# African-Robotics-Unit/AcinoSet

Measured on AMD Instinct MI355X. Metric: FTE frames/sec (residual+Jac+LM step), 6-cam x 20-joint, higher is better.
Workload: dtype f64

## Files before the change

### acinoset_amd/csrc/chunk.hip

```cpp
#include "chunk.hpp"

#include <algorithm>
#include <cstdlib>
#include <type_traits>

#include "bcr_dev.hpp"
#include "trio80.hpp"

namespace acino {

void ChunkPlan::build(int nodes_total, int chunk_nodes, bool pin_l, bool pin_r) {
  n_nodes = nodes_total;
  m = n_chunks = n_sep = 0;
  node0 = pin_l ? 1 : 0;
  pin_right = pin_r ? 1 : 0;
  const int nodes = nodes_total - node0;
  if (chunk_nodes < 0 || nodes < 1) return;
  int mm = chunk_nodes;
  if (mm == 0) {
    mm = (nodes + 255) / 256;
    mm = std::max(4, std::min(mm, 512));
  }
  mm = std::max(2, mm);
  m = mm;
  n_chunks = (nodes + mm - 1) / mm;
  if (pin_r && n_chunks > 1 && nodes - (n_chunks - 1) * mm == 1) --n_chunks;
  n_sep = n_chunks - 1 + node0 + pin_right;
}

__device__ __forceinline__ void tile_store(double* M, int ib, int jb, const d4& a, int li, int lk) {
#pragma unroll
  for (int rr = 0; rr < 4; ++rr) M[(ib * 16 + lk + 4 * rr) * LD + jb * 16 + li] = a[rr];
}

constexpr int SW_VEC = 18 * NP + 2 * BS + 8 + 8 + 3 * NP + 64;
static constexpr size_t kSweepLds = (3 * MAT + SW_VEC) * sizeof(double);

__device__ __forceinline__ int opaque(int x) {
  asm volatile("" : "+v"(x));
  return x;
}

__device__ __forceinline__ unsigned opaque_u(unsigned x) {
  asm volatile("" : "+v"(x));
  return x;
}
struct BuildSlot {
  int pr, pc, base, e;
  bool own, dg;
  static __device__ __forceinline__ BuildSlot unpack(unsigned w) {
    BuildSlot s;
    s.pr = w & 31;
    s.pc = (w >> 5) & 31;
    s.own = (w >> 10) & 1;
    s.dg = (w >> 11) & 1;
    s.base = (w >> 12) & 2047;
    s.e = w >> 23;
    return s;
  }
};
static_assert((NP - 1) * LD + NP - 1 < 2048 && 13 * NP <= 512 && NP <= 32, "BuildSlot's bit fields");

constexpr int SW_T = 512;
template <int NQ>
__device__ __forceinline__ void syrk_mask_n(d4 (&acc)[NQ], bool load) {
#pragma unroll
  for (int q = 0; q < NQ; ++q)
#pragma unroll
    for (int rr = 0; rr < 4; ++rr) acc[q][rr] = load ? acc[q][rr] : 0.0;
}
constexpr int SP_STEPS = 4 * NT - 1;
__device__ __forceinline__ void spike_gf(const double* G, const double (&bF)[NT][4], d4 (&acc)[NT], int li, int lk) {
  double a[3][NT];
  const double* gb = G + lk * LD + li;
  auto fetch = [&](int buf, int step) {
#pragma unroll
    for (int ib = 0; ib < NT; ++ib) a[buf][ib] = gb[(4 * step) * LD + ib * 16];
  };
#pragma unroll
  for (int ib = 0; ib < NT; ++ib) acc[ib] = d4{0, 0, 0, 0};
  fetch(0, 0);
  fetch(1, 1);
#pragma unroll
  for (int step = 0; step < SP_STEPS; ++step) {
    if (step + 2 < SP_STEPS) fetch((step + 2) % 3, step + 2);
    __builtin_amdgcn_sched_barrier(0);
#pragma unroll
    for (int ib = 0; ib < NT; ++ib) acc[ib] = mfma(a[step % 3][ib], bF[step >> 2][step & 3], acc[ib]);
    __builtin_amdgcn_sched_barrier(0);
  }
}
template <int NQ>
__device__ __forceinline__ void spike_ftt(d4 (&acc)[NQ], const double* Yf, const d4 (&T)[NT], const int (&as)[NQ], int li, int lk) {
  constexpr int DEPTH = NQ >= 3 ? 2 : (NQ == 2 ? 3 : 6);
  const double* p = Yf + lk * LD + li;
  double a[DEPTH + 1][NQ];
#pragma unroll
  for (int d = 0; d < DEPTH; ++d)
#pragma unroll
    for (int q = 0; q < NQ; ++q) a[d][q] = p[(4 * d) * LD + as[q] * 16];
#pragma unroll
  for (int st = 0; st < SP_STEPS; ++st) {
    if (st + DEPTH < SP_STEPS) {
#pragma unroll
      for (int q = 0; q < NQ; ++q) a[(st + DEPTH) % (DEPTH + 1)][q] = p[(4 * (st + DEPTH)) * LD + as[q] * 16];
    }
    __builtin_amdgcn_sched_barrier(0);
#pragma unroll
    for (int q = 0; q < NQ; ++q) acc[q] = mfma(-a[st % (DEPTH + 1)][q], T[st >> 2][st & 3], acc[q]);
    __builtin_amdgcn_sched_barrier(0);
  }
}
template <int NQ>
struct AlTiles {
  d4 acc[NQ];
  int as[NQ], j;
  double* Ag;
  __device__ __forceinline__ double* at(int q, int rr, int li, int lk) const {
    return as[q] >= j ? Ag + (size_t)(as[q] * 16 + 4 * rr + lk) * BS + j * 16 + li
                      : Ag + (size_t)(j * 16 + li) * BS + as[q] * 16 + 4 * rr + lk;
  }
  __device__ __forceinline__ void fetch(int li, int lk) {
#pragma unroll
    for (int q = 0; q < NQ; ++q)
#pragma unroll
      for (int rr = 0; rr < 4; ++rr) acc[q][rr] = *at(q, rr, li, lk);
  }
  __device__ __forceinline__ void run(bool load, const double* Yf, const d4 (&T)[NT], int li, int lk) {
    syrk_mask_n<NQ>(acc, load);
    spike_ftt<NQ>(acc, Yf, T, as, li, lk);
#pragma unroll
    for (int q = 0; q < NQ; ++q)
#pragma unroll
      for (int rr = 0; rr < 4; ++rr) *at(q, rr, li, lk) = acc[q][rr];
  }
};
__device__ __forceinline__ int role8(int wave) { return (0x75236410u >> (4 * wave)) & 15; }
constexpr int ctri_i(int t) { return (t >= 1) + (t >= 3) + (t >= 6) + (t >= 10); }
template <int T>
struct GramTile {
  static constexpr int ib = ctri_i(T), jb = T - ib * (ib + 1) / 2, ns = 4 * (NT - ib);
};
template <int T>
__device__ __forceinline__ void gram_fetch(const double* X, int li, int lk, double (&a)[GramTile<T>::ns], double (&b)[GramTile<T>::ns]) {
  const double* pa = X + (GramTile<T>::ib * 16 + li) * LD + GramTile<T>::ib * 16 + lk;
  const double* pb = X + (GramTile<T>::jb * 16 + li) * LD + GramTile<T>::ib * 16 + lk;
#pragma unroll
  for (int s = 0; s < GramTile<T>::ns; ++s) {
    a[s] = pa[4 * s];
    b[s] = pb[4 * s];
  }
}
template <int T>
__device__ __forceinline__ void gram_tile(double* Xg, int li, int lk, const double (&a)[GramTile<T>::ns], const double (&b)[GramTile<T>::ns]) {
  constexpr int ib = GramTile<T>::ib, jb = GramTile<T>::jb;
  d4 g = {0, 0, 0, 0};
#pragma unroll
  for (int s = 0; s < GramTile<T>::ns; ++s) g = mfma(a[s], b[s], g);
#pragma unroll
  for (int rr = 0; rr < 4; ++rr) {
    Xg[(ib * 16 + lk + 4 * rr) * LD + jb * 16 + li] = g[rr];
    if (ib != jb) Xg[(jb * 16 + li) * LD + ib * 16 + lk + 4 * rr] = g[rr];
  }
}
template <int T0, int... REST>
__device__ __forceinline__ void gram_chain(const double* Xf, double* Xg, int li, int lk, const double (&a)[GramTile<T0>::ns],
                                           const double (&b)[GramTile<T0>::ns]) {
  if constexpr (sizeof...(REST) > 0) {
    constexpr int rest[] = {REST...};
    double an[GramTile<rest[0]>::ns], bn[GramTile<rest[0]>::ns];
    gram_fetch<rest[0]>(Xf, li, lk, an, bn);
    __builtin_amdgcn_sched_barrier(0);
    gram_tile<T0>(Xg, li, lk, a, b);
    __builtin_amdgcn_sched_barrier(0);
    gram_chain<REST...>(Xf, Xg, li, lk, an, bn);
  } else {
    gram_tile<T0>(Xg, li, lk, a, b);
  }
}
template <int T0, int... REST>
__device__ __forceinline__ void gram_fixed(const double* Xf, double* Xg, int* done, int li, int lk, int lane) {
  double a[GramTile<T0>::ns], b[GramTile<T0>::ns];
  gram_fetch<T0>(Xf, li, lk, a, b);
  gram_chain<T0, REST...>(Xf, Xg, li, lk, a, b);
  asm volatile("" ::: "memory");
  if (lane == 0) __hip_atomic_fetch_add(done, 1 + (int)sizeof...(REST), __ATOMIC_RELAXED, __HIP_MEMORY_SCOPE_WORKGROUP);
  asm volatile("" ::: "memory");
}

struct SpikeArgs {
  const double* Xg;
  double* Y;
  double* Ag;
  const double* cRk;
  const double* bvn;
  double* zk;
  double *Cg, *bR;
  int *c_gfdone, *c_fready, *c_bv, *tdone;
  int *g_open, *g_done;
  const double* Xf;
  int k, n_s;
  bool hasL, has_next;
  long long* stamps;
};
template <int ROLE>
__device__ __forceinline__ void spike_node(const SpikeArgs& A, int& tsb, int ln) {
  constexpr bool two = ROLE == 5;
  constexpr int j0 = ROLE == 4 ? 1 : (ROLE == 5 ? 2 : (ROLE == 6 ? 3 : 4));
  constexpr int NA = ROLE == 4 ? 3 : (ROLE == 5 ? 2 : (ROLE == 6 ? 5 : 4));
  const int li = ln & 15, lk = ln >> 4;
  double* const Y = A.Y;
  auto stamp = [&](int i) { if (A.stamps && ln == 0) A.stamps[i] = (long long)wall_clock64(); };
  AlTiles<NA> al;
  AlTiles<1> al0;
  al.Ag = A.Ag;
  al.j = j0;
  if (ROLE == 4) { al.as[0] = 1; al.as[1] = 0; al.as[2 % NA] = 2; }
  if (ROLE == 5) { al.as[0] = 2; al.as[1] = 0; }
  if (ROLE == 6) { al.as[0] = 3; al.as[1] = 0; al.as[2 % NA] = 1; al.as[3 % NA] = 2; al.as[4 % NA] = 4; }
  if (ROLE == 7) { al.as[0] = 4; al.as[1] = 0; al.as[2 % NA] = 1; al.as[3 % NA] = 2; }
  al0.Ag = A.Ag;
  al0.j = 0;
  al0.as[0] = 0;
  if (A.hasL) {
    al.fetch(li, lk);
    if (two) al0.fetch(li, lk);
  }
  if (ROLE >= 6) {
    double* const Xg = const_cast<double*>(A.Xg);
    lds_wait(A.g_open, A.k + 1);
    if (ROLE == 6) gram_fixed<2, 13>(A.Xf, Xg, A.g_done, li, lk, ln);
    else if (A.hasL) gram_fixed<5, 9, 14>(A.Xf, Xg, A.g_done, li, lk, ln);
    else gram_fixed<2, 5, 9, 13, 14>(A.Xf, Xg, A.g_done, li, lk, ln);
  }
  lds_wait(A.g_done, 15 * (A.k + 1));
  stamp(16 + 4 * (ROLE - 4));
  d4 T0[NT], T1[NT];
  {
    double bF[NT][4];
    const double* yb = Y + lk * LD + j0 * 16 + li;
#pragma unroll
    for (int kb = 0; kb < NT; ++kb)
#pragma unroll
      for (int s = 0; s < 4; ++s) bF[kb][s] = (4 * kb + s < SP_STEPS) ? yb[(kb * 16 + 4 * s) * LD] : 0.0;
    spike_gf(A.Xg, bF, T0, li, lk);
  }
  if (two) {
    double bF[NT][4];
    const double* yb = Y + lk * LD + li;
#pragma unroll
    for (int kb = 0; kb < NT; ++kb)
#pragma unroll
      for (int s = 0; s < 4; ++s) bF[kb][s] = (4 * kb + s < SP_STEPS) ? yb[(kb * 16 + 4 * s) * LD] : 0.0;
    spike_gf(A.Xg, bF, T1, li, lk);
  }
  lds_signal(A.c_gfdone, ln);
  stamp(17 + 4 * (ROLE - 4));
  if (A.hasL) {
    lds_wait(A.c_fready, A.n_s * A.k);
    al.run(A.k > 0, Y, T0, li, lk);
    if (two) al0.run(A.k > 0, Y, T1, li, lk);
  }
  stamp(18 + 4 * (ROLE - 4));
  if (A.hasL) {
    if (ROLE != 5) lds_signal(A.tdone + (ROLE == 4 ? 0 : (ROLE == 6 ? 1 : 2)), ln);
    if (ROLE == 7 || ROLE == 4 || ROLE == 5) lds_wait(A.tdone + 1, A.k + 1);
    if (ROLE == 4 || ROLE == 5) lds_wait(A.tdone + 2, A.k + 1);
    if (ROLE == 5) lds_wait(A.tdone + 0, A.k + 1);
  }
  (void)tsb;
#pragma unroll
  for (int ib = 0; ib < NT; ++ib) tile_store(Y, ib, j0, T0[ib], li, lk);
  if (two) {
#pragma unroll
    for (int ib = 0; ib < NT; ++ib) tile_store(Y, ib, 0, T1[ib], li, lk);
  }
  if (ROLE == 7) {
    A.zk[ln] = Y[ln * LD + (BS - 1)];
    if (ln < 16) A.zk[64 + ln] = Y[(64 + ln) * LD + (BS - 1)];
  }
  if (A.has_next) {
    lds_wait(A.c_bv, A.k + 1);
    const double* const cRk = A.cRk;
    const double* const bvn = A.bvn;
    const int p = ln % NP, cg = ln / NP;
#pragma unroll
    for (int h = 0; h < (two ? 2 : 1); ++h) {
      const int c_lo = 16 * (h ? 0 : j0);
      if (cg < 2) {
        const double e00 = cRk[(0 * 3 + 0) * NP + p], e01 = cRk[(0 * 3 + 1) * NP + p], e02 = cRk[(0 * 3 + 2) * NP + p];
        const double e11 = cRk[(1 * 3 + 1) * NP + p], e12 = cRk[(1 * 3 + 2) * NP + p], e22 = cRk[(2 * 3 + 2) * NP + p];
        const double b0 = bvn[p], b1 = bvn[NP + p], b2 = bvn[2 * NP + p];
        double fv[8][3];
#pragma unroll
        for (int q = 0; q < 8; ++q) {
          const int cc = c_lo + cg + 2 * q;
          fv[q][0] = Y[p * LD + cc];
          fv[q][1] = Y[(NP + p) * LD + cc];
          fv[q][2] = Y[(2 * NP + p) * LD + cc];
        }
#pragma unroll
        for (int q = 0; q < 8; ++q) {
          const int cc = c_lo + cg + 2 * q;
          const double f0 = fv[q][0], f1 = fv[q][1], f2 = fv[q][2];
          double o0 = -(e00 * f0 + e01 * f1 + e02 * f2), o1 = -(e11 * f1 + e12 * f2), o2 = -(e22 * f2);
          if (cc == BS - 1) {
            o0 += b0;
            o1 += b1;
            o2 += b2;
          }
          Y[p * LD + cc] = o0;
          Y[(NP + p) * LD + cc] = o1;
          Y[(2 * NP + p) * LD + cc] = o2;
        }
      }
      if (ln < 16)
        for (int r = 3 * NP; r < BS; ++r) Y[r * LD + c_lo + ln] = 0.0;
    }
  }
  lds_signal(A.c_fready, ln);
  stamp(19 + 4 * (ROLE - 4));
  if (A.bR) {
    if (A.Cg && !two) {
      const int cc = 16 * j0 + li;
#pragma unroll 5
      for (int r = lk; r < BS; r += 4) A.Cg[r * BS + cc] = cc < 3 * NP ? Y[r * LD + cc] : 0.0;
    }
    if (ROLE == 7) {
      A.bR[ln] = Y[ln * LD + (BS - 1)];
      if (ln < 16) A.bR[64 + ln] = Y[(64 + ln) * LD + (BS - 1)];
    }
  }
}


__global__ void __launch_bounds__(SW_T)
k_chunk_sweep(BcrChain ch, SepView sp, const FteConst* __restrict__ cst, int* numeric_err, const int* __restrict__ status,
                int m, int n_chunks, int node0, int pin_right) {
  extern __shared__ __attribute__((aligned(16))) char smem_raw[];
  if (status && *status != 0) return;
  double* const Xf = reinterpret_cast<double*>(smem_raw);
  double* const Xg = Xf + MAT;
  double* const Y = Xg + MAT;
  double* const cL = Y + MAT;
  double* const cR0 = cL + 9 * NP;
  double* const bvb = cR0 + 9 * NP;
  double* const red = bvb + 2 * BS;
  int* const sync = reinterpret_cast<int*>(red + 8);
  int* const cB = sync + 5;
  int* const tdone = sync + 2;
  int* const g_done = sync + 6;
  int* const g_open = sync + 10;
  int* const c_gfdone = sync + 7;
  int* const c_fready = sync + 8;
  int* const c_bv = sync + 9;
  double* const kq = red + 16;
  double* const klo = kq + NP;
  double* const khi = klo + NP;
  long long* const lst = reinterpret_cast<long long*>(khi + NP);
  const int tid = threadIdx.x, wave = tid >> 6, lane = tid & 63;
  const FteConst& K = *cst;
  const int c = blockIdx.x;
  const int first = node0 + c * m;
  const bool hasL = c > 0 || node0 > 0, hasR = c + 1 < n_chunks || pin_right;
  const int len = c + 1 < n_chunks ? m : ch.n_nodes - first;
  const int n_int = hasR ? len - 1 : len;
  const int sL = c - 1 + node0, sR = c + node0;
  const size_t MB = (size_t)BS * BS;
  const int role = __builtin_amdgcn_readfirstlane(role8(wave));
  const TableGeom TG = table_geom(K);
  const bool left_int = left_table_is_interior(TG, first);
  int tab_cur = 0;
  bool tab_int0 = right_table_is_interior(TG, first), tab_int1 = left_int;
  const int n_s = hasL ? 4 : 1;
  const bool builder = role <= 3;
  const bool strips = role >= 4 && (hasL || role == 7);
  double gmax_run = 0.0;
  long long* const dbgp = (ch.dbg && (long long)blockIdx.x == ch.dbg[64] && ch.dbg[66] == 0) ? ch.dbg : nullptr;
  const int dbg_k = dbgp ? (int)ch.dbg[65] : -1;
  if (dbgp && lane == 0) {
    const unsigned hw = __builtin_amdgcn_s_getreg((31 << 11) | 4);
    atomicOr(reinterpret_cast<unsigned long long*>(ch.dbg + 67), (unsigned long long)((hw >> 4) & 3) << (4 * wave));
    if (wave == 0) ch.dbg[68] = hw;
  }
#define SW_STAMP(i) do { if (dbgp && k == dbg_k && lane == 0) lst[i] = (long long)wall_clock64(); } while (0)
  if (tid < 16) sync[tid] = 0;
  if (tid < 64) lst[tid] = 0;
  if (dbgp && tid == 0) dbgp[70] = (long long)wall_clock64();
  if (c == 0 && node0) {
    for (int e = tid; e < BS * BS; e += SW_T) sp.D[e] = 0.0;
    if (tid < BS) sp.b[tid] = 0.0;
  }
  if (tid < NP) {
    kq[tid] = K.q_w[tid];
    klo[tid] = K.lo[tid];
    khi[tid] = K.hi[tid];
  }
  __syncthreads();

  TrioSync tsy;
  {
    NodeFetch f;
    build_fetch<SW_T>(f, ch, K, first, tid);
    if (left_int && tab_int0) {
      if (tid < 2 * 9 * NP) {
        const int q = tid % (9 * NP), pair = q / NP, p = q % NP, ii = pair / 3, jj = pair % 3;
        cL[tid] = ii <= jj ? 2.0 * kq[p] * (jj == ii ? -1.0 : (jj - ii == 1 ? 6.0 : -15.0)) : 0.0;
      }
    } else {
      fill_coupling_coef<SW_T>(cL, cR0, K, first, tid, kq);
    }
    for (int e = tid; e < MAT; e += SW_T) Y[e] = 0.0;
    gmax_run = build_finish<SW_T>(Xf, bvb, f, K, first, tid, kq, klo, khi);
    __syncthreads();
    if (dbgp && tid == 0) lst[60] = (long long)wall_clock64();
    if (hasL)
      for (int e = tid; e < 9 * NP; e += SW_T) {
        const int pair = e / NP, p = e % NP, ii = pair / 3, jj = pair % 3;
        if (ii <= jj) Y[(ii * NP + p) * LD + jj * NP + p] = cL[e];
      }
    if (tid < BS) Y[tid * LD + (BS - 1)] = bvb[tid];
    __syncthreads();
    if (role < 3) chol80_trio(Xf, role, lane, numeric_err, sync, tsy);
    __syncthreads();
    if (dbgp && tid == 0) lst[61] = (long long)wall_clock64();
  }

  unsigned slot0 = 0, slot1 = 0;
  if (builder) {
    auto pack = [](int e, bool own, bool dg) {
      const int pa = e / 13, dd = e % 13, pc = pa + dd >= NP ? pa + dd - NP : pa + dd;
      return (unsigned)pa | (unsigned)pc << 5 | (unsigned)own << 10 | (unsigned)dg << 11 | (unsigned)(pa * LD + pc) << 12 | (unsigned)e << 23;
    };
    auto offdiag = [](int n) { return 13 * (n / 12) + 1 + n % 12; };
    const bool dg0 = role == 1 && lane < NP;
    const int n0 = role == 1 ? 192 + lane - NP : (role == 0 ? 0 : (role == 2 ? 64 : 128)) + lane;
    slot0 = pack(dg0 ? 13 * lane : offdiag(n0), true, dg0);
    const bool own1 = (role == 3 && lane < 35) || (role == 2 && lane < 34);
    slot1 = pack(own1 ? offdiag((role == 3 ? 231 : 266) + lane) : 0, own1, false);
  }
  int tb = 0, tsb = 0;
#pragma unroll 1
  for (int k = 0; k < n_int; ++k) {
    const int node = first + k, next = node + 1;
    const bool last = k + 1 == n_int;
    const bool has_next = !last || hasR;
    const int ln = opaque(lane);
    const int li = ln & 15, lk = ln >> 4;
    bool tab_write = false, tab_interior = false;
    if (k > 0) {
      tab_interior = right_table_is_interior(TG, node);
      if (!(tab_interior && (tab_cur ? tab_int1 : tab_int0))) {
        tab_cur ^= 1;
        tab_write = !(tab_interior && (tab_cur ? tab_int1 : tab_int0));
        if (tab_cur) tab_int1 = tab_interior;
        else tab_int0 = tab_interior;
      }
    }
    double* const cRk = tab_cur ? cL : cR0;
    if (builder) {
      const int bw = role;
      const int bt = bw * 64 + ln;
      const int fb_next = 3 * (next - node0);
      const BuildSlot s0 = BuildSlot::unpack(opaque_u(slot0)), s1 = BuildSlot::unpack(opaque_u(slot1));
      const bool two = bw >= 2;
      double hq[2][3] = {{0, 0, 0}, {0, 0, 0}}, xq[3] = {0, 0, 0}, gq[3] = {0, 0, 0}, cvq[3] = {0, 0, 0}, lamq = 0.0;
      bool liveq[3] = {false, false, false}, ownq[3] = {false, false, false};
      if (has_next) {
        const int cur = ch.st->cur;
        const double* Hg = cur ? ch.H1 : ch.H0;
        lamq = ch.st->lam;
#pragma unroll
        for (int j = 0; j < 3; ++j)
          if (fb_next + j < K.n_frames) {
            hq[0][j] = Hg[(size_t)(fb_next + j) * HPAIRS + s0.e];
            if (two && s1.own) hq[1][j] = Hg[(size_t)(fb_next + j) * HPAIRS + s1.e];
          }
        if (s0.dg) {
          const int pdg = s0.pr;
          const double* xg = cur ? ch.x1 : ch.x0;
          const double* gg = cur ? ch.g1 : ch.g0;
#pragma unroll
          for (int j = 0; j < 3; ++j)
            if (fb_next + j < K.n_frames) {
              xq[j] = xg[(size_t)(fb_next + j + HALO) * NP + pdg];
              gq[j] = gg[(size_t)(fb_next + j) * NP + pdg];
            }
#pragma unroll
          for (int pr = 0; pr < 3; ++pr) {
            const int j = pr == 2 ? 1 : 0, jp = pr == 0 ? 1 : 2;
            if (fb_next + jp < K.n_frames)
              cvq[pr] = 2.0 * kq[pdg] * band_coef_clip(K.n_offset + fb_next + j, jp - j, K.n_global, K.clip_len);
          }
        }
#pragma unroll
        for (int j = 0; j < 3; ++j) {
          liveq[j] = fb_next + j < K.n_frames;
          ownq[j] = fb_next + j >= K.own_lo && fb_next + j < K.own_hi;
        }
      }
      if (bw == 0) SW_STAMP(0);
      lds_barrier(cB, tb, 4, ln);
      lds_wait(c_gfdone, n_s * k);
      if (bw == 0) SW_STAMP(1);
      if (bt == 0) __hip_atomic_fetch_add(g_open, 1, __ATOMIC_RELAXED, __HIP_MEMORY_SCOPE_WORKGROUP);
      if (tab_write) {
        if (tab_interior) right_table_interior<256>(cRk, bt, [&](int p) { return kq[p]; });
        else fill_coupling_coef<256>(nullptr, cRk, K, node, bt, kq);
      }
      if (bw == 0) gram_fixed<0, 10>(Xf, Xg, g_done, li, lk, ln);
      else if (bw == 1) gram_fixed<1, 7>(Xf, Xg, g_done, li, lk, ln);
      else if (bw == 2) gram_fixed<4, 8, 12>(Xf, Xg, g_done, li, lk, ln);
      else gram_fixed<3, 6, 11>(Xf, Xg, g_done, li, lk, ln);
      SW_STAMP(32 + wave);
      lds_barrier(cB, tb, 4, ln);
      lds_wait(g_done, 15 * (k + 1));
      if (bw == 0) SW_STAMP(2);
#pragma unroll
      for (int j = 0; j < 3; ++j) asm volatile("" : "+v"(hq[0][j]), "+v"(hq[1][j]), "+v"(xq[j]), "+v"(gq[j]));
      asm volatile("" : "+v"(lamq));
      if (has_next) {
        double* const bvn = bvb + ((k + 1) & 1) * BS;
        double ca[2][6], cb[2][6], gv[2][3][3];
        auto slot_reads = [&](const BuildSlot& sl, double (&a)[6], double (&b)[6], double (&g)[3][3]) {
          const double *ta = cRk + sl.pr, *tb_ = cRk + sl.pc;
          a[0] = ta[0 * NP]; a[1] = ta[1 * NP]; a[2] = ta[2 * NP];
          a[3] = ta[4 * NP]; a[4] = ta[5 * NP]; a[5] = ta[8 * NP];
          b[0] = tb_[0 * NP]; b[1] = tb_[1 * NP]; b[2] = tb_[2 * NP];
          b[3] = tb_[4 * NP]; b[4] = tb_[5 * NP]; b[5] = tb_[8 * NP];
          const double* gp0 = Xg + sl.base;
#pragma unroll
          for (int jj = 0; jj < 3; ++jj) {
            const double* gp = gp0 + jj * NP * LD;
            g[jj][0] = gp[0];
            g[jj][1] = gp[NP];
            g[jj][2] = gp[2 * NP];
          }
        };
        auto slot_finish = [&](const BuildSlot& sl, auto may_diag, const double (&a)[6], const double (&b)[6], const double (&g)[3][3],
                               const double (&h)[3]) {
#pragma clang fp contract(off)
          constexpr bool DIAG = decltype(may_diag)::value;
          const int pr = sl.pr;
          const bool dg = DIAG && sl.dg;
          const double a00 = a[0], a01 = a[1], a02 = a[2], a11 = a[3], a12 = a[4], a22 = a[5];
          const double b00 = b[0], b01 = b[1], b02 = b[2], b11 = b[3], b12 = b[4], b22 = b[5];
          double mm[3][3], S[2][3];
#pragma unroll
          for (int jj = 0; jj < 3; ++jj) {
            const double g0 = g[jj][0], g1 = g[jj][1], g2 = g[jj][2];
            mm[jj][0] = __builtin_fma(g2, b02, __builtin_fma(g0, b00, g1 * b01));
            mm[jj][1] = __builtin_fma(g1, b11, g2 * b12);
            mm[jj][2] = g2 * b22;
          }
#pragma unroll
          for (int ii = 0; ii < 3; ++ii) {
            S[0][ii] = __builtin_fma(a02, mm[2][ii], __builtin_fma(a00, mm[0][ii], a01 * mm[1][ii]));
            S[1][ii] = __builtin_fma(a11, mm[1][ii], a12 * mm[2][ii]);
          }
          double v[3][3];
#pragma unroll
          for (int j = 0; j < 3; ++j)
#pragma unroll
            for (int jp = 0; jp < 3; ++jp) v[j][jp] = (j == jp ? h[j] : 0.0);
          if (dg) {
#pragma unroll
            for (int j = 0; j < 3; ++j) {
              double d = 1.0, bb = 0.0;
              if (liveq[j]) {
                d = h[j];
                const double gtol = GRAD_ZERO_REL * d;
                const bool fixed = (xq[j] <= klo[pr] && gq[j] > gtol) || (xq[j] >= khi[pr] && gq[j] < -gtol);
                d = __builtin_fma(lamq, fmax(d, DIAG_FLOOR), d);
                if (fixed) d *= FIX_SCALE;
                bb = fixed ? 0.0 : -gq[j];
                if (ownq[j]) gmax_run = fmax(gmax_run, fabs(bb));
              }
              v[j][j] = d;
              bvn[j * NP + pr] = bb;
            }
            v[0][1] = v[1][0] = cvq[0];
            v[0][2] = v[2][0] = cvq[1];
            v[1][2] = v[2][1] = cvq[2];
          }
          double val[3][3];
#pragma unroll
          for (int jp = 0; jp < 3; ++jp) {
            val[0][jp] = v[0][jp] - S[0][jp];
            val[1][jp] = v[1][jp] - S[1][jp];
          }
          val[2][0] = __builtin_fma(-a22, mm[2][0], v[2][0]);
          val[2][1] = v[2][1] - a22 * mm[2][1];
          val[2][2] = __builtin_fma(-a22, mm[2][2], v[2][2]);
          if (sl.own) {
            double* const xa = Xf + sl.base;
            double* const xt = Xf + sl.pc * LD + pr;
#pragma unroll
            for (int j = 0; j < 3; ++j)
#pragma unroll
              for (int jp = 0; jp < 3; ++jp) {
                xa[j * NP * LD + jp * NP] = val[j][jp];
                if (!dg) xt[jp * NP * LD + j * NP] = val[j][jp];
              }
          }
        };
        const BuildSlot b0 = BuildSlot::unpack(opaque_u(slot0)), b1 = BuildSlot::unpack(opaque_u(slot1));
        slot_reads(b0, ca[0], cb[0], gv[0]);
        slot_finish(b0, std::true_type{}, ca[0], cb[0], gv[0], hq[0]);
        if (two) {
          slot_reads(b1, ca[1], cb[1], gv[1]);
          slot_finish(b1, std::false_type{}, ca[1], cb[1], gv[1], hq[1]);
        }
        if (bt < BS - 3 * NP) {
          Xf[(3 * NP + bt) * LD + 3 * NP + bt] = 1.0;
          bvn[3 * NP + bt] = 0.0;
        }
      }
      lds_barrier(cB, tb, 4, ln);
      if (bt == 0) __hip_atomic_fetch_add(c_bv, 1, __ATOMIC_RELAXED, __HIP_MEMORY_SCOPE_WORKGROUP);
      if (bw == 0) SW_STAMP(4);
      if (bw < 3) {
        if (!last) {
          chol80_trio<false>(Xf, bw, ln, numeric_err, sync, tsy, (dbgp && k == dbg_k) ? lst : nullptr);
        } else if (hasR) {
          double2* d2 = reinterpret_cast<double2*>(sp.D + (size_t)sR * MB);
          for (int idx = bt; idx < BS * BS / 2; idx += 192) {
            const int e = 2 * idx, r = e / BS, cc = e % BS;
            d2[idx] = make_double2(Xf[r * LD + cc], Xf[r * LD + cc + 1]);
          }
          if (hasL) {
            double* const Cg = sp.Cpl + (size_t)sL * MB;
            lds_wait(c_fready, n_s * (k + 1));
#pragma unroll 7
            for (int idx = bt; idx < 2 * BS * 8; idx += 192) {
              const int h = idx / (BS * 8), rem = idx % (BS * 8), r = rem >> 3, cc = (h ? 32 : 0) + 2 * (rem & 7);
              *reinterpret_cast<double2*>(Cg + r * BS + cc) = make_double2(Y[r * LD + cc], Y[r * LD + cc + 1]);
            }
          }
        }
        SW_STAMP(8 + wave);
      } else if (bw == 3) {
        double* Gg = ch.D + node * MB;
#pragma unroll 6
        for (int q = 0; q < LOWER_ITEMS / 64; ++q) {
          const int idx = ln + 64 * q;
          int r, cc;
          lower_item(idx, r, cc);
          *reinterpret_cast<double2*>(Gg + r * BS + cc) = make_double2(Xg[r * LD + cc], Xg[r * LD + cc + 1]);
        }
        SW_STAMP(8 + wave);
      }
    }
    if (strips) {
      SpikeArgs sa;
      sa.Xg = Xg; sa.Y = Y; sa.Ag = sp.AL + (size_t)(hasL ? opaque(sL) : 0) * MB; sa.cRk = cRk; sa.bvn = bvb + ((k + 1) & 1) * BS;
      sa.zk = ch.b + (size_t)node * BS; sa.g_open = g_open; sa.g_done = g_done; sa.Xf = Xf; sa.c_gfdone = c_gfdone; sa.c_fready = c_fready; sa.c_bv = c_bv; sa.tdone = tdone;
      sa.bR = (last && hasR) ? sp.b + (size_t)sR * BS : nullptr;
      sa.Cg = (last && hasR && hasL) ? sp.Cpl + (size_t)sL * MB : nullptr;
      sa.k = k; sa.n_s = n_s; sa.hasL = hasL; sa.has_next = has_next; sa.stamps = (dbgp && k == dbg_k) ? lst : nullptr;
      if (role == 4) spike_node<4>(sa, tsb, ln);
      else if (role == 5) spike_node<5>(sa, tsb, ln);
      else if (role == 6) spike_node<6>(sa, tsb, ln);
      else spike_node<7>(sa, tsb, ln);
    }
  }
  __syncthreads();
  if (dbgp) {
    if (tid == 0) lst[62] = (long long)wall_clock64();
    __syncthreads();
    if (tid < 64 && lst[tid]) dbgp[tid] = lst[tid];
  }
#undef SW_STAMP
  publish_gmax<SW_T>(gmax_run, red, ch.gn_part, c, tid);
  if (dbgp && tid == 0) dbgp[71] = (long long)wall_clock64();
}

__global__ void __launch_bounds__(256) k_sep_combine(SepView sp, const int* __restrict__ status) {
  if (status && *status != 0) return;
  const int q = blockIdx.x, tid = threadIdx.x;
  const size_t MB = (size_t)BS * BS;
  double* D = sp.D + q * MB;
  const double* A = sp.AL + q * MB;
  constexpr int NQ = (LOWER_ITEMS + 255) / 256;
  double2 dv[NQ], av[NQ];
  const double bq = tid < 3 * NP ? sp.b[(size_t)q * BS + tid] : 0.0, aq = tid < 3 * NP ? A[(size_t)(BS - 1) * BS + tid] : 0.0;
#pragma unroll
  for (int k = 0; k < NQ; ++k) {
    const int idx = tid + 256 * k;
    if (idx < LOWER_ITEMS) {
      int r, cc;
      lower_item(idx, r, cc);
      dv[k] = *reinterpret_cast<const double2*>(D + r * BS + cc);
      av[k] = *reinterpret_cast<const double2*>(A + r * BS + cc);
    }
  }
#pragma unroll
  for (int k = 0; k < NQ; ++k) {
    const int idx = tid + 256 * k;
    if (idx < LOWER_ITEMS) {
      int r, cc;
      lower_item(idx, r, cc);
      if (r < 3 * NP) {
        const double ax = cc < 3 * NP ? av[k].x : 0.0, ay = cc + 1 < 3 * NP ? av[k].y : 0.0;
        *reinterpret_cast<double2*>(D + r * BS + cc) = make_double2(dv[k].x + ax, dv[k].y + ay);
      }
    }
  }
  if (tid < 3 * NP) sp.b[(size_t)q * BS + tid] = bq + aq;
}

constexpr int BK_PW = 4;
constexpr int BK_NL = 4;
constexpr int BK_T = 64 * (BK_PW + BK_NL);
constexpr int BK_NB = 2;
constexpr int BLD = 82;
constexpr int BK_Q = LOWER_ITEMS / 64;
constexpr int BK_FL = 8;
static_assert(LOWER_ITEMS == 64 * NT * (NT + 1), "30 rounds of 64 items: 2 (ib + 1) per tile row");
static_assert(BK_FL >= BK_NL + BK_NB + 2, "a far f_k must have been stored (and waited for) before a loader asks for it");
constexpr int BK_OPS = BS * BLD, BK_TAB = BK_OPS + 5 * BS, BK_STAGE = BK_TAB + 9 * NP + 1;
static constexpr size_t kBacksubLds =
    (BK_NB * BK_STAGE + 2 * BS + BK_FL * BS + 2 * 9 * NP + 16 + NP + 1) * sizeof(double) + 16 * sizeof(int);

typedef double d2 __attribute__((ext_vector_type(2)));
template <int CTRL>
__device__ __forceinline__ double dpp_add(double v) {
  const long long b = __double_as_longlong(v);
  const int lo = __builtin_amdgcn_update_dpp(0, (int)b, CTRL, 0xf, 0xf, false);
  const int hi = __builtin_amdgcn_update_dpp(0, (int)(b >> 32), CTRL, 0xf, 0xf, false);
  return v + __longlong_as_double(((long long)hi << 32) | (unsigned)lo);
}
__device__ __forceinline__ double lanes8_sum(double v) {
  v = dpp_add<0x141>(v);
  v = dpp_add<0xB1>(v);
  return dpp_add<0x4E>(v);
}
__global__ void __launch_bounds__(BK_T)
k_chunk_backsub(BcrChain ch, SepView sp, const FteConst* __restrict__ cst, const int* __restrict__ status, int m,
                int n_chunks, int node0, int pin_right, TrialOut trial) {
  extern __shared__ __attribute__((aligned(16))) char smem_raw[];
  double* const stg = reinterpret_cast<double*>(smem_raw);
  double* const ub = stg + BK_NB * BK_STAGE;
  double* const fl = ub + 2 * BS;
  double* const cL0 = fl + BK_FL * BS;
  double* const cRl = cL0 + 9 * NP;
  double* const red = cRl + 9 * NP;
  double* const kq = red + 16;
  int* const sync = reinterpret_cast<int*>(kq + NP + 1);
  int* const c_ready = sync;
  int* const c_rd = sync + BK_NL;
  int* const c_u = sync + BK_NL + 1;
  const int tid = threadIdx.x, lane = tid & 63, wave = tid >> 6;
  const int c = blockIdx.x, first = node0 + c * m;
  const bool hasL = c > 0 || node0 > 0, hasR = c + 1 < n_chunks || pin_right;
  const int len = c + 1 < n_chunks ? m : ch.n_nodes - first;
  const int n_int = hasR ? len - 1 : len;
  const int sL = c - 1 + node0, sR = c + node0;
  const size_t MB = (size_t)BS * BS;
  const int nf = hasL && n_int > 0 ? n_int - 1 : 0;
  const int ns = nf + n_int;
  auto node_at = [&](int s) __attribute__((always_inline)) { return s < nf ? s : n_int - 1 - (s - nf); };
  struct Rounds {
    int row0[BK_Q], col0[BK_Q];
    constexpr Rounds() : row0{}, col0{} {
      int q = 0;
      for (int ib = 0; ib < NT; ++ib)
        for (int h = 0; h < 2; ++h)
          for (int jc = 0; jc <= ib; ++jc) {
            row0[q] = 16 * ib + 8 * h;
            col0[q] = 16 * jc;
            ++q;
          }
    }
  };
  constexpr Rounds RD{};
  const int gl = (lane >> 3) * BS + 2 * (lane & 7), ll = (lane >> 3) * BLD + 2 * (lane & 7);
  d2 g[BK_Q];
  const int gl74 = ((lane >> 3) < 3 ? (lane >> 3) : 2) * BS + 2 * (lane & 7);
  auto tile_fetch = [&](int k) __attribute__((always_inline)) {
    const double* G = ch.D + (size_t)(first + k) * MB;
#pragma unroll
    for (int q = 0; q < BK_Q; ++q)
      g[q] = *reinterpret_cast<const d2*>(G + (RD.row0[q] * BS + RD.col0[q]) + (RD.row0[q] + 8 > 3 * NP ? gl74 : gl));
  };
  const int lw = wave - BK_PW;
  if (lw >= 0 && lw < ns) tile_fetch(node_at(lw));
  if (status && *status != 0) return;
  const FteConst& K = *cst;
  const bool uni = coupling_tables_uniform(K, first, first + n_int - 1);
  auto table_node = [&](int s) __attribute__((always_inline)) {
    const int k = node_at(s);
    return s < nf ? k : (k > 0 ? k - 1 : 0);
  };
  const int t_cur = ch.st->cur, t_nf = K.n_frames;
  const double* t_x = t_cur ? ch.x1 : ch.x0;
  const double* t_g = t_cur ? ch.g1 : ch.g0;
  const double* t_hd = t_cur ? trial.hd1 : trial.hd0;
  double* const fst = ch.Wl + (size_t)first * BS;
  if (ch.dbg && (long long)blockIdx.x == ch.dbg[64] && ch.dbg[66] == 1 && tid == 0) ch.dbg[61] = (long long)wall_clock64();
  if (c == 0 && sp.flags) {
    for (int e = tid; e < sp.n_flags; e += BK_T) sp.flags[e] = 0;
    if (tid == 0) sp.flags[sp.n_flags] += 1;
  }
  if (tid < 16) sync[tid] = 0;
  if (tid < 2 * BS) ub[tid] = 0.0;
  if (tid < NP) kq[tid] = K.q_w[tid];
  fill_coupling_coef<BK_T>(cL0, nullptr, K, first, tid);
  fill_coupling_coef<BK_T>(nullptr, cRl, K, first + (n_int > 0 ? n_int - 1 : 0), tid);
  double t_pred = 0.0, t_step = 0.0;
  if (wave >= BK_PW) {
    constexpr int NRO = (5 * 3 * NP + 63) / 64;
    double ro[NRO];
    auto ro_fetch = [&](int t) __attribute__((always_inline)) {
      if (t < nf) return;
      const int k = node_at(t), node = first + k;
      const bool far = hasL && k >= 1 && n_int - k >= BK_FL;
// ... 287 lines not shown
```

### acinoset_amd/csrc/trio80.hpp

```cpp
#pragma once
#include "dense80.hpp"

namespace acino {

__device__ __forceinline__ void lds_signal(int* f, int lane) {
  asm volatile("" ::: "memory");
  if (lane == 0) __hip_atomic_fetch_add(f, 1, __ATOMIC_RELAXED, __HIP_MEMORY_SCOPE_WORKGROUP);
  asm volatile("" ::: "memory");
}
__device__ __forceinline__ void lds_wait(int* f, int target) {
  while (__hip_atomic_load(f, __ATOMIC_RELAXED, __HIP_MEMORY_SCOPE_WORKGROUP) < target) __builtin_amdgcn_s_sleep(1);
  asm volatile("" ::: "memory");
}
__device__ __forceinline__ void lds_wait2(int* f0, int t0, int* f1, int t1) {
  for (;;) {
    const int a = __hip_atomic_load(f0, __ATOMIC_RELAXED, __HIP_MEMORY_SCOPE_WORKGROUP);
    const int b = __hip_atomic_load(f1, __ATOMIC_RELAXED, __HIP_MEMORY_SCOPE_WORKGROUP);
    if (a >= t0 && b >= t1) break;
    __builtin_amdgcn_s_sleep(1);
  }
  asm volatile("" ::: "memory");
}
__device__ __forceinline__ void lds_barrier(int* cnt, int& target, int n, int lane) {
  target += n;
  lds_signal(cnt, lane);
  lds_wait(cnt, target);
}

template <int KB, int R0 = KB + 2, int R1 = NT - 1>
struct LowerList {
  int ti[9], tj[9], n;
  constexpr LowerList() : ti{}, tj{}, n(0) {
    for (int r = R0; r <= R1; ++r)
      for (int c = KB + 1; c <= r; ++c) {
        ti[n] = r;
        tj[n] = c;
        ++n;
      }
  }
};
template <int KB>
struct UpperList {
  int ti[16], tj[16], n;
  constexpr UpperList() : ti{}, tj{}, n(0) {
    for (int r = 0; r <= KB; ++r)
      for (int c = KB + 1; c < NT; ++c) {
        ti[n] = r;
        tj[n] = c;
        ++n;
      }
  }
};
template <class LIST, int KB, int Q0, int NQ>
__device__ __forceinline__ void trail_run(double* Lm, const double (&P)[NT][4], int li, int lk) {
  constexpr LIST TL{};
  d4 a[NQ];
#pragma unroll
  for (int q = 0; q < NQ; ++q) {
    const int ti = TL.ti[Q0 + q], tj = TL.tj[Q0 + q];
    const double* Cc = Lm + (ti * 16) * LD + tj * 16;
#pragma unroll
    for (int rr = 0; rr < 4; ++rr) a[q][rr] = ti == KB ? 0.0 : Cc[(lk + 4 * rr) * LD + li];
  }
#pragma unroll
  for (int s = 0; s < 4; ++s) {
#pragma unroll
    for (int q = 0; q < NQ; ++q) a[q] = mfma(-P[TL.ti[Q0 + q]][s], P[TL.tj[Q0 + q]][s], a[q]);
  }
#pragma unroll
  for (int q = 0; q < NQ; ++q) {
    double* Cc = Lm + (TL.ti[Q0 + q] * 16) * LD + TL.tj[Q0 + q] * 16;
#pragma unroll
    for (int rr = 0; rr < 4; ++rr) Cc[(lk + 4 * rr) * LD + li] = a[q][rr];
  }
}
template <class LIST, int KB, int Q0>
__device__ __forceinline__ void trail_rest(double* Lm, const double (&P)[NT][4], int li, int lk) {
  constexpr LIST TL{};
  if constexpr (Q0 < TL.n) {
    constexpr int NQ = TL.n - Q0 < 4 ? TL.n - Q0 : 4;
    trail_run<LIST, KB, Q0, NQ>(Lm, P, li, lk);
    trail_rest<LIST, KB, Q0 + NQ>(Lm, P, li, lk);
  }
}
template <int KB>
__device__ __forceinline__ void load_panel(double (&P)[NT][4], const double* Lm, int li, int lk) {
#pragma unroll
  for (int t = 0; t < NT; ++t)
#pragma unroll
    for (int s = 0; s < 4; ++s) P[t][s] = Lm[(t * 16 + li) * LD + KB * 16 + 4 * s + lk];
}
template <int KB, class LIST = LowerList<KB>>
__device__ __forceinline__ void helperL_trailing(double* Lm, int li, int lk, int* ccrit, int lane) {
  constexpr LIST TL{};
  double P[NT][4];
  d4 a[TL.n];
  load_panel<KB>(P, Lm, li, lk);
#pragma unroll
  for (int q = 0; q < TL.n; ++q) {
    const double* Cc = Lm + (TL.ti[q] * 16) * LD + TL.tj[q] * 16;
#pragma unroll
    for (int rr = 0; rr < 4; ++rr) a[q][rr] = Cc[(lk + 4 * rr) * LD + li];
  }
  constexpr int NC = TL.n < 2 ? TL.n : 2;
#pragma unroll
  for (int s = 0; s < 4; ++s)
#pragma unroll
    for (int q = 0; q < NC; ++q) a[q] = mfma(-P[TL.ti[q]][s], P[TL.tj[q]][s], a[q]);
#pragma unroll
  for (int q = 0; q < NC; ++q) {
    double* Cc = Lm + (TL.ti[q] * 16) * LD + TL.tj[q] * 16;
#pragma unroll
    for (int rr = 0; rr < 4; ++rr) Cc[(lk + 4 * rr) * LD + li] = a[q][rr];
  }
  lds_signal(ccrit, lane);
#pragma unroll
  for (int s = 0; s < 4; ++s)
#pragma unroll
    for (int q = NC; q < TL.n; ++q) a[q] = mfma(-P[TL.ti[q]][s], P[TL.tj[q]][s], a[q]);
#pragma unroll
  for (int q = NC; q < TL.n; ++q) {
    double* Cc = Lm + (TL.ti[q] * 16) * LD + TL.tj[q] * 16;
#pragma unroll
    for (int rr = 0; rr < 4; ++rr) Cc[(lk + 4 * rr) * LD + li] = a[q][rr];
  }
}
template <int KB>
__device__ __forceinline__ void helperU_trailing(double* Lm, int li, int lk) {
  double P[NT][4];
  load_panel<KB>(P, Lm, li, lk);
  trail_rest<UpperList<KB>, KB, 0>(Lm, P, li, lk);
}
template <int NQ>
__device__ __forceinline__ void panel_tiles(double* Lm, int kb, int t0, int li, int lk) {
  const double* Ukk = Lm + (kb * 16) * LD + kb * 16;
  double bq[4], av[NQ][4];
  d4 acc[NQ];
#pragma unroll
  for (int s = 0; s < 4; ++s) bq[s] = Ukk[(4 * s + lk) * LD + li];
#pragma unroll
  for (int q = 0; q < NQ; ++q) {
    const double* A = Lm + ((t0 + q) * 16) * LD + kb * 16;
#pragma unroll
    for (int s = 0; s < 4; ++s) av[q][s] = A[li * LD + 4 * s + lk];
    acc[q] = d4{0, 0, 0, 0};
  }
#pragma unroll
  for (int s = 0; s < 4; ++s)
#pragma unroll
    for (int q = 0; q < NQ; ++q) acc[q] = mfma(av[q][s], bq[s], acc[q]);
#pragma unroll
  for (int q = 0; q < NQ; ++q) {
    double* A = Lm + ((t0 + q) * 16) * LD + kb * 16;
#pragma unroll
    for (int rr = 0; rr < 4; ++rr) A[(lk + 4 * rr) * LD + li] = acc[q][rr];
  }
}
struct TrioSync {
  int t3 = 0, posts = 0, crit = 0, lpan = 0, udone = 0, ulow = 0;
};
template <bool MEET = true>
__device__ __forceinline__ void chol80_trio(double* Lm, int role, int lane, int* err, int* sync, TrioSync& ts,
                                             long long* dbg = nullptr) {
  const int li = lane & 15, lk = lane >> 4;
  int* const c3 = sync;
  int* const ccrit = sync + 12;
  int* const cpost = sync + 13;
  int* const clpan = sync + 14;
  int* const cudone = sync + 15;
  int* const culow = sync + 11;
  const int post0 = ts.posts, crit0 = ts.crit, lp0 = ts.lpan;
  if (role == 0) {
    __builtin_amdgcn_s_setprio(3);
    chol16_inv(Lm, lane, err);
    lds_signal(cpost, lane);
#pragma unroll 1
    for (int kb = 0; kb < NT - 1; ++kb) {
      if (kb > 0) lds_wait(ccrit, crit0 + kb);
      panel_tiles<1>(Lm, kb, kb + 1, li, lk);
      lds_signal(cpost, lane);
      if (dbg && lane == 0) dbg[40 + 2 * kb] = (long long)wall_clock64();
      double* Cc = Lm + ((kb + 1) * 16) * LD + (kb + 1) * 16;
      const double* A = Lm + ((kb + 1) * 16) * LD + kb * 16;
      d4 a;
      double av[4];
#pragma unroll
      for (int rr = 0; rr < 4; ++rr) a[rr] = Cc[(lk + 4 * rr) * LD + li];
#pragma unroll
      for (int s = 0; s < 4; ++s) av[s] = A[li * LD + 4 * s + lk];
#pragma unroll
      for (int s = 0; s < 4; ++s) a = mfma(-av[s], av[s], a);
      chol16_inv_acc(Cc, a, lane, err);
      lds_signal(cpost, lane);
      if (dbg && lane == 0) dbg[41 + 2 * kb] = (long long)wall_clock64();
    }
    lds_wait(cudone, ts.udone + 1);
    panel_tiles<1>(Lm, NT - 1, 0, li, lk);
    __builtin_amdgcn_s_setprio(0);
  } else if (role == 1) {
    __builtin_amdgcn_s_setprio(2);
#pragma unroll 1
    for (int kb = 0; kb < NT - 1; ++kb) {
      lds_wait(cpost, post0 + 2 * kb + 1);
      if (kb == 1) lds_wait(culow, ts.ulow + 1);
      if (kb == 0) panel_tiles<3>(Lm, 0, 2, li, lk);
      else if (kb == 1) panel_tiles<2>(Lm, 1, 3, li, lk);
      else if (kb == 2) panel_tiles<1>(Lm, 2, 4, li, lk);
      lds_signal(clpan, lane);
      lds_wait(cpost, post0 + 2 * kb + 2);
      if (dbg && lane == 0) dbg[56 + kb] = (long long)wall_clock64();
      if (kb == 0) helperL_trailing<0, LowerList<0, 2, 3>>(Lm, li, lk, ccrit, lane);
      else if (kb == 1) helperL_trailing<1>(Lm, li, lk, ccrit, lane);
      else if (kb == 2) helperL_trailing<2>(Lm, li, lk, ccrit, lane);
      else lds_signal(ccrit, lane);
      if (dbg && lane == 0) dbg[48 + kb] = (long long)wall_clock64();
    }
    lds_wait(cpost, post0 + 2 * (NT - 1) + 1);
    lds_wait(cudone, ts.udone + 1);
    panel_tiles<2>(Lm, NT - 1, 1, li, lk);
    __builtin_amdgcn_s_setprio(0);
  } else {
    __builtin_amdgcn_s_setprio(1);
#pragma unroll 1
    for (int kb = 0; kb < NT - 1; ++kb) {
      lds_wait(cpost, post0 + 2 * kb + 1);
      if (kb == 1) panel_tiles<1>(Lm, 1, 0, li, lk);
      else if (kb == 2) panel_tiles<2>(Lm, 2, 0, li, lk);
      else if (kb == 3) panel_tiles<3>(Lm, 3, 0, li, lk);
      lds_wait(cpost, post0 + 2 * kb + 2);
      lds_wait(clpan, lp0 + kb + 1);
      if (kb == 0) {
        double P[NT][4];
        load_panel<0>(P, Lm, li, lk);
        trail_rest<LowerList<0, 4, 4>, 0, 0>(Lm, P, li, lk);
        lds_signal(culow, lane);
        trail_rest<UpperList<0>, 0, 0>(Lm, P, li, lk);
      } else if (kb == 1) helperU_trailing<1>(Lm, li, lk);
      else if (kb == 2) helperU_trailing<2>(Lm, li, lk);
      else helperU_trailing<3>(Lm, li, lk);
      if (dbg && lane == 0) dbg[52 + kb] = (long long)wall_clock64();
    }
    lds_signal(cudone, lane);
    lds_wait(cpost, post0 + 2 * (NT - 1) + 1);
    panel_tiles<1>(Lm, NT - 1, 3, li, lk);
    __builtin_amdgcn_s_setprio(0);
  }
  if (MEET) lds_barrier(c3, ts.t3, 3, lane);
  ts.posts = post0 + 9;
  ts.crit = crit0 + 4;
  ts.lpan = lp0 + 4;
  ts.udone += 1;
  ts.ulow += 1;
}


}
```

Baseline: 25.34 million.

## Spread last-node spike work across idle builder waves in chunk sweep

On the last node of a chunk with a left separator, the spike update work that wave roles 5 and 6 used to do is now split across builder waves 0 and 1 (new roles 9 and 10). The Gram store and separator-diagonal store move to the freed waves, and handover goes through a new LDS counter with agent-scope atomic loads of the AL tiles. The initial Cholesky wave assignment is also changed so that role 4 runs the third trio lane while role 2 only advances its sync counters. The aim is to shorten the critical path of the final node by balancing work across waves, at the cost of extra synchronisation complexity and a risk of deadlocks or ordering bugs.

```diff
diff --git a/acinoset_amd/csrc/chunk.hip b/acinoset_amd/csrc/chunk.hip
--- a/acinoset_amd/csrc/chunk.hip
+++ b/acinoset_amd/csrc/chunk.hip
@@ -125,6 +125,12 @@
     for (int q = 0; q < NQ; ++q)
 #pragma unroll
       for (int rr = 0; rr < 4; ++rr) acc[q][rr] = *at(q, rr, li, lk);
+  }
+  __device__ __forceinline__ void fetch_handed_over(int li, int lk) {
+#pragma unroll
+    for (int q = 0; q < NQ; ++q)
+#pragma unroll
+      for (int rr = 0; rr < 4; ++rr) acc[q][rr] = __hip_atomic_load(at(q, rr, li, lk), __ATOMIC_RELAXED, __HIP_MEMORY_SCOPE_AGENT);
   }
   __device__ __forceinline__ void run(bool load, const double* Yf, const d4 (&T)[NT], int li, int lk) {
     syrk_mask_n<NQ>(acc, load);
@@ -198,16 +204,32 @@
   double *Cg, *bR;
   int *c_gfdone, *c_fready, *c_bv, *tdone;
   int *g_open, *g_done;
+  int* c_end;
   const double* Xf;
   int k, n_s;
   bool hasL, has_next;
   long long* stamps;
 };
+__device__ __forceinline__ void store_G(const double* Xg, double* Gg, int ln) {
+#pragma unroll 6
+  for (int q = 0; q < LOWER_ITEMS / 64; ++q) {
+    const int idx = ln + 64 * q;
+    int r, cc;
+    lower_item(idx, r, cc);
+    *reinterpret_cast<double2*>(Gg + r * BS + cc) = make_double2(Xg[r * LD + cc], Xg[r * LD + cc + 1]);
+  }
+}
+__device__ __forceinline__ void hand_over(int* c_end, int ln) {
+  asm volatile("s_waitcnt vmcnt(0)" ::: "memory");
+  lds_signal(c_end, ln);
+}
 template <int ROLE>
 __device__ __forceinline__ void spike_node(const SpikeArgs& A, int& tsb, int ln) {
   constexpr bool two = ROLE == 5;
-  constexpr int j0 = ROLE == 4 ? 1 : (ROLE == 5 ? 2 : (ROLE == 6 ? 3 : 4));
-  constexpr int NA = ROLE == 4 ? 3 : (ROLE == 5 ? 2 : (ROLE == 6 ? 5 : 4));
+  constexpr bool moved = ROLE >= 9;
+  constexpr int j0 = ROLE == 4 ? 1 : (ROLE == 5 || ROLE == 8 ? 2 : (ROLE == 6 || ROLE == 10 ? 3 : (ROLE == 7 ? 4 : 0)));
+  constexpr int NA = ROLE == 4 ? 3 : (ROLE == 5 || ROLE == 8 ? 2 : (ROLE == 6 || ROLE == 10 ? 5 : (ROLE == 7 ? 4 : 1)));
+  constexpr int sb = ROLE <= 7 ? 16 + 4 * (ROLE - 4) : (ROLE == 8 ? 20 : (ROLE == 9 ? 40 : 44));
   const int li = ln & 15, lk = ln >> 4;
   double* const Y = A.Y;
   auto stamp = [&](int i) { if (A.stamps && ln == 0) A.stamps[i] = (long long)wall_clock64(); };
@@ -216,17 +238,22 @@
   al.Ag = A.Ag;
   al.j = j0;
   if (ROLE == 4) { al.as[0] = 1; al.as[1] = 0; al.as[2 % NA] = 2; }
-  if (ROLE == 5) { al.as[0] = 2; al.as[1] = 0; }
-  if (ROLE == 6) { al.as[0] = 3; al.as[1] = 0; al.as[2 % NA] = 1; al.as[3 % NA] = 2; al.as[4 % NA] = 4; }
+  if (ROLE == 5 || ROLE == 8) { al.as[0] = 2; al.as[1 % NA] = 0; }
+  if (ROLE == 6 || ROLE == 10) { al.as[0] = 3; al.as[1 % NA] = 0; al.as[2 % NA] = 1; al.as[3 % NA] = 2; al.as[4 % NA] = 4; }
   if (ROLE == 7) { al.as[0] = 4; al.as[1] = 0; al.as[2 % NA] = 1; al.as[3 % NA] = 2; }
+  if (ROLE == 9) al.as[0] = 0;
   al0.Ag = A.Ag;
   al0.j = 0;
   al0.as[0] = 0;
-  if (A.hasL) {
+  if (ROLE == 8) hand_over(A.c_end, ln);
+  if (moved) {
+    lds_wait2(A.c_end, 2, A.c_fready, A.n_s * A.k);
+    al.fetch_handed_over(li, lk);
+  } else if (A.hasL) {
     al.fetch(li, lk);
     if (two) al0.fetch(li, lk);
   }
-  if (ROLE >= 6) {
+  if (ROLE == 6 || ROLE == 7) {
     double* const Xg = const_cast<double*>(A.Xg);
     lds_wait(A.g_open, A.k + 1);
     if (ROLE == 6) gram_fixed<2, 13>(A.Xf, Xg, A.g_done, li, lk, ln);
@@ -234,7 +261,7 @@
     else gram_fixed<2, 5, 9, 13, 14>(A.Xf, Xg, A.g_done, li, lk, ln);
   }
   lds_wait(A.g_done, 15 * (A.k + 1));
-  stamp(16 + 4 * (ROLE - 4));
+  stamp(sb + 0);
   d4 T0[NT], T1[NT];
   {
     double bF[NT][4];
@@ -255,18 +282,23 @@
     spike_gf(A.Xg, bF, T1, li, lk);
   }
   lds_signal(A.c_gfdone, ln);
-  stamp(17 + 4 * (ROLE - 4));
+  stamp(sb + 1);
   if (A.hasL) {
     lds_wait(A.c_fready, A.n_s * A.k);
     al.run(A.k > 0, Y, T0, li, lk);
     if (two) al0.run(A.k > 0, Y, T1, li, lk);
   }
-  stamp(18 + 4 * (ROLE - 4));
+  stamp(sb + 2);
   if (A.hasL) {
-    if (ROLE != 5) lds_signal(A.tdone + (ROLE == 4 ? 0 : (ROLE == 6 ? 1 : 2)), ln);
-    if (ROLE == 7 || ROLE == 4 || ROLE == 5) lds_wait(A.tdone + 1, A.k + 1);
-    if (ROLE == 4 || ROLE == 5) lds_wait(A.tdone + 2, A.k + 1);
-    if (ROLE == 5) lds_wait(A.tdone + 0, A.k + 1);
+    if (ROLE == 4 || ROLE == 6 || ROLE == 7 || ROLE == 10) lds_signal(A.tdone + (ROLE == 4 ? 0 : (ROLE == 7 ? 2 : 1)), ln);
+    if (ROLE == 8) {
+      lds_wait(A.c_end, 2);
+      lds_signal(A.c_end, ln);
+    }
+    if (ROLE == 7 || ROLE == 4 || ROLE == 5 || ROLE == 8 || ROLE == 9) lds_wait(A.tdone + 1, A.k + 1);
+    if (ROLE == 4 || ROLE == 5 || ROLE == 8 || ROLE == 9) lds_wait(A.tdone + 2, A.k + 1);
+    if (ROLE == 5 || ROLE == 8 || ROLE == 9) lds_wait(A.tdone + 0, A.k + 1);
+    if (ROLE == 9) lds_wait(A.c_end, 3);
   }
   (void)tsb;
 #pragma unroll
@@ -319,7 +351,7 @@
     }
   }
   lds_signal(A.c_fready, ln);
-  stamp(19 + 4 * (ROLE - 4));
+  stamp(sb + 3);
   if (A.bR) {
     if (A.Cg && !two) {
       const int cc = 16 * j0 + li;
@@ -351,6 +383,7 @@
   int* const tdone = sync + 2;
   int* const g_done = sync + 6;
   int* const g_open = sync + 10;
+  int* const c_end = sync + 1;
   int* const c_gfdone = sync + 7;
   int* const c_fready = sync + 8;
   int* const c_bv = sync + 9;
@@ -421,7 +454,8 @@
       }
     if (tid < BS) Y[tid * LD + (BS - 1)] = bvb[tid];
     __syncthreads();
-    if (role < 3) chol80_trio(Xf, role, lane, numeric_err, sync, tsy);
+    if (role < 2 || role == 4) chol80_trio(Xf, role == 4 ? 2 : role, lane, numeric_err, sync, tsy, (dbgp && dbg_k < 0) ? lst : nullptr);
+    else if (role == 2) tsy.sat_out(true);
     __syncthreads();
     if (dbgp && tid == 0) lst[61] = (long long)wall_clock64();
   }
@@ -458,6 +492,17 @@
       }
     }
     double* const cRk = tab_cur ? cL : cR0;
+    const bool spread = last && hasL;
+    auto spike_args = [&]() {
+      SpikeArgs sa;
+      sa.Xg = Xg; sa.Y = Y; sa.Ag = sp.AL + (size_t)(hasL ? opaque(sL) : 0) * MB; sa.cRk = cRk; sa.bvn = bvb + ((k + 1) & 1) * BS;
+      sa.zk = ch.b + (size_t)node * BS; sa.g_open = g_open; sa.g_done = g_done; sa.Xf = Xf; sa.c_gfdone = c_gfdone; sa.c_fready = c_fready; sa.c_bv = c_bv; sa.tdone = tdone;
+      sa.c_end = c_end;
+      sa.bR = (last && hasR) ? sp.b + (size_t)sR * BS : nullptr;
+      sa.Cg = (last && hasR && hasL) ? sp.Cpl + (size_t)sL * MB : nullptr;
+      sa.k = k; sa.n_s = n_s; sa.hasL = hasL; sa.has_next = has_next; sa.stamps = (dbgp && k == dbg_k) ? lst : nullptr;
+      return sa;
+    };
     if (builder) {
       const int bw = role;
       const int bt = bw * 64 + ln;
@@ -619,49 +664,53 @@
       lds_barrier(cB, tb, 4, ln);
       if (bt == 0) __hip_atomic_fetch_add(c_bv, 1, __ATOMIC_RELAXED, __HIP_MEMORY_SCOPE_WORKGROUP);
       if (bw == 0) SW_STAMP(4);
+      auto store_sep_diag = [&](int part, int parts) {
+        double2* d2 = reinterpret_cast<double2*>(sp.D + (size_t)sR * MB);
+        for (int idx = 64 * part + ln; idx < BS * BS / 2; idx += 64 * parts) {
+          const int e = 2 * idx, r = e / BS, cc = e % BS;
+          d2[idx] = make_double2(Xf[r * LD + cc], Xf[r * LD + cc + 1]);
+        }
+      };
       if (bw < 3) {
         if (!last) {
           chol80_trio<false>(Xf, bw, ln, numeric_err, sync, tsy, (dbgp && k == dbg_k) ? lst : nullptr);
-        } else if (hasR) {
-          double2* d2 = reinterpret_cast<double2*>(sp.D + (size_t)sR * MB);
-          for (int idx = bt; idx < BS * BS / 2; idx += 192) {
-            const int e = 2 * idx, r = e / BS, cc = e % BS;
-            d2[idx] = make_double2(Xf[r * LD + cc], Xf[r * LD + cc + 1]);
-          }
-          if (hasL) {
-            double* const Cg = sp.Cpl + (size_t)sL * MB;
-            lds_wait(c_fready, n_s * (k + 1));
-#pragma unroll 7
-            for (int idx = bt; idx < 2 * BS * 8; idx += 192) {
-              const int h = idx / (BS * 8), rem = idx % (BS * 8), r = rem >> 3, cc = (h ? 32 : 0) + 2 * (rem & 7);
-              *reinterpret_cast<double2*>(Cg + r * BS + cc) = make_double2(Y[r * LD + cc], Y[r * LD + cc + 1]);
-            }
-          }
+        } else if (!spread) {
+          if (hasR) store_sep_diag(bw, 3);
+        } else if (bw == 2) {
+          if (hasR) store_sep_diag(0, 2);
+        } else {
+          if (dbgp && k == dbg_k && ln == 0) lst[63] = (long long)wall_clock64();
+          const SpikeArgs sa = spike_args();
+          if (bw == 0) spike_node<10>(sa, tsb, ln);
+          else spike_node<9>(sa, tsb, ln);
         }
         SW_STAMP(8 + wave);
       } else if (bw == 3) {
-        double* Gg = ch.D + node * MB;
-#pragma unroll 6
-        for (int q = 0; q < LOWER_ITEMS / 64; ++q) {
-          const int idx = ln + 64 * q;
-          int r, cc;
-          lower_item(idx, r, cc);
-          *reinterpret_cast<double2*>(Gg + r * BS + cc) = make_double2(Xg[r * LD + cc], Xg[r * LD + cc + 1]);
-        }
+        if (!spread) store_G(Xg, ch.D + node * MB, ln);
+        else if (hasR) store_sep_diag(1, 2);
         SW_STAMP(8 + wave);
       }
     }
     if (strips) {
-      SpikeArgs sa;
-      sa.Xg = Xg; sa.Y = Y; sa.Ag = sp.AL + (size_t)(hasL ? opaque(sL) : 0) * MB; sa.cRk = cRk; sa.bvn = bvb + ((k + 1) & 1) * BS;
-      sa.zk = ch.b + (size_t)node * BS; sa.g_open = g_open; sa.g_done = g_done; sa.Xf = Xf; sa.c_gfdone = c_gfdone; sa.c_fready = c_fready; sa.c_bv = c_bv; sa.tdone = tdone;
-      sa.bR = (last && hasR) ? sp.b + (size_t)sR * BS : nullptr;
-      sa.Cg = (last && hasR && hasL) ? sp.Cpl + (size_t)sL * MB : nullptr;
-      sa.k = k; sa.n_s = n_s; sa.hasL = hasL; sa.has_next = has_next; sa.stamps = (dbgp && k == dbg_k) ? lst : nullptr;
+      const SpikeArgs sa = spike_args();
       if (role == 4) spike_node<4>(sa, tsb, ln);
-      else if (role == 5) spike_node<5>(sa, tsb, ln);
-      else if (role == 6) spike_node<6>(sa, tsb, ln);
-      else spike_node<7>(sa, tsb, ln);
+      else if (role == 5) {
+        if (spread) spike_node<8>(sa, tsb, ln);
+        else spike_node<5>(sa, tsb, ln);
+      } else if (role == 6) {
+        if (spread) {
+          hand_over(c_end, ln);
+          lds_wait(g_open, k + 1);
+          gram_fixed<2, 13>(Xf, Xg, g_done, li, lk, ln);
+          lds_wait(g_done, 15 * (k + 1));
+          store_G(Xg, ch.D + node * MB, ln);
+          if (dbgp && k == dbg_k && ln == 0) lst[24] = (long long)wall_clock64();
+        } else {
+          spike_node<6>(sa, tsb, ln);
+        }
+      } else {
+        spike_node<7>(sa, tsb, ln);
+      }
     }
   }
   __syncthreads();
diff --git a/acinoset_amd/csrc/trio80.hpp b/acinoset_amd/csrc/trio80.hpp
--- a/acinoset_amd/csrc/trio80.hpp
+++ b/acinoset_amd/csrc/trio80.hpp
@@ -158,6 +158,14 @@
 }
 struct TrioSync {
   int t3 = 0, posts = 0, crit = 0, lpan = 0, udone = 0, ulow = 0;
+  __device__ __forceinline__ void sat_out(bool meet) {
+    if (meet) t3 += 3;
+    posts += 9;
+    crit += 4;
+    lpan += 4;
+    udone += 1;
+    ulow += 1;
+  }
 };
 template <bool MEET = true>
 __device__ __forceinline__ void chol80_trio(double* Lm, int role, int lane, int* err, int* sync, TrioSync& ts,
```

After: 25.63 million (median of 6 runs). 1.1% higher.
